# naver-ai/egtr

Hardware: AMD Instinct MI355X
Metric: images/sec end-to-end SGG, 600x1000 input, N=200 queries (higher is better)
Workload: dtype f32; 1 GPU; VG inference: ResNet-50, N=200, 6 enc/6 dec, 150 classes, 50 predicates, 600x1000, bs=1/GPU fp32 (BASELINE configs[1]); hip_graph=True, gemm_tuning=True, miopen_find=True, parallelism=replicas x1 (independent images, no collective)

## Files before the change

egtr_amd/csrc/ffn_x6.hip:

```cpp
#include <hip/hip_runtime.h>
#include <stdint.h>

#include "common.h"
#include "x6_common.h"
#include "xs_format.h"

namespace {
using namespace x6;

constexpr int kD = 256;
constexpr int kRows = 64;
constexpr int kKS = kD / 16;
constexpr int kFrag = xs::kFragBytes;
constexpr int kPanel = 2 * kKS * 2 * kFrag;
constexpr int kHbuf = 2 * 4 * 3 * kFrag;
constexpr int kStage = 24 * kFrag;
constexpr int kLds = kPanel + kHbuf + 3 * kStage;
static_assert(kLds == 160 * 1024, "the whole LDS of a CU");
constexpr int NL = 6;
typedef float f32x8 __attribute__((ext_vector_type(8)));

struct FfnArgs {
  const float* x;
  const float* res;
  const char* w1;
  const float* b1;
  const char* w2;
  const float* b2;
  const float* gamma;
  const float* beta;
  const float* pos;
  float* out;
  float* out_pos;
  int M, ldx, ldr, F, pos_rows;
  float eps;
  const char* wp;
  const float* bp;
  const float* gamma1;
  const float* beta1;
  float eps1;
};

__device__ __forceinline__ int swz(int x, int ks) { return x ^ (ks & 15) ^ ((x >> 5) << 2); }

__device__ __forceinline__ void build_panel(const float* __restrict__ x, int ldx, int M, int r0, int tid, int lane,
                                            char* panel, char* lo0, char* lo1) {
  float4 v[16];
#pragma unroll
  for (int it = 0; it < 16; ++it) {
    const int row = min(r0 + it * 4 + (tid >> 6), M - 1);
    v[it] = *reinterpret_cast<const float4*>(x + (size_t)row * ldx + 4 * lane);
  }
#pragma unroll
  for (int it = 0; it < 16; ++it) {
    const int row = it * 4 + (tid >> 6), rb = row >> 5, r = row & 31;
    const int ks = lane >> 2, off = (swz(r + 32 * ((lane >> 1) & 1), ks) << 4) + (lane & 1) * 8;
    const xs::Split3 s0 = xs::split3_fast(v[it].x), s1 = xs::split3_fast(v[it].y), s2 = xs::split3_fast(v[it].z),
                     s3 = xs::split3_fast(v[it].w);
    char* p = panel + ((rb * kKS + ks) * 2) * kFrag + off;
    *reinterpret_cast<uint2*>(p) = make_uint2(xs::pack_hi16(s0.hi, s1.hi), xs::pack_hi16(s2.hi, s3.hi));
    *reinterpret_cast<uint2*>(p + kFrag) = make_uint2(xs::pack_hi16(s0.mid, s1.mid), xs::pack_hi16(s2.mid, s3.mid));
    char* q = (rb == 0 ? lo0 : lo1) + ks * kFrag + off;
    *reinterpret_cast<uint2*>(q) = make_uint2(xs::pack_hi16(s0.lo, s1.lo), xs::pack_hi16(s2.lo, s3.lo));
  }
}

template <bool USE_RES_OF, class ResFn>
__device__ __forceinline__ void final_epilogue(const f32x16 (&acc2)[4], const FfnArgs& A, int r0, int wave, int lane,
                                               float* red, ResFn&& res_of) {
  const int wm = wave >> 1, wn = wave & 1, li = lane & 31, hf = lane >> 5;
  const int row = r0 + wm * 32 + li;
  float4 y[4][4];
#pragma unroll
  for (int t = 0; t < 4; ++t)
#pragma unroll
    for (int q = 0; q < 4; ++q) {
      const int col = (4 * wn + t) * 32 + 8 * q + 4 * hf;
      const float4 b = A.b2 != nullptr ? *reinterpret_cast<const float4*>(A.b2 + col) : make_float4(0.f, 0.f, 0.f, 0.f);
      y[t][q] = make_float4(acc2[t][4 * q + 0] + b.x, acc2[t][4 * q + 1] + b.y, acc2[t][4 * q + 2] + b.z,
                            acc2[t][4 * q + 3] + b.w);
    }
  if (A.gamma != nullptr) {
    const float* xr = A.res + (size_t)min(row, A.M - 1) * A.ldr;
#pragma unroll
    for (int t = 0; t < 4; ++t)
#pragma unroll
      for (int q = 0; q < 4; ++q) {
        float4 r;
        if constexpr (USE_RES_OF) r = res_of(t, q);
        else r = *reinterpret_cast<const float4*>(xr + (4 * wn + t) * 32 + 8 * q + 4 * hf);
        y[t][q].x += r.x; y[t][q].y += r.y; y[t][q].z += r.z; y[t][q].w += r.w;
      }
    __syncthreads();
    float sum = 0.f;
#pragma unroll
    for (int t = 0; t < 4; ++t)
#pragma unroll
      for (int q = 0; q < 4; ++q) sum += (y[t][q].x + y[t][q].y) + (y[t][q].z + y[t][q].w);
    sum += __shfl_xor(sum, 32);
    if (hf == 0) red[wave * 32 + li] = sum;
    __syncthreads();
    const float mean = (sum + red[(wave ^ 1) * 32 + li]) * (1.f / kD);
    float sq = 0.f;
#pragma unroll
    for (int t = 0; t < 4; ++t)
#pragma unroll
      for (int q = 0; q < 4; ++q) {
        y[t][q].x -= mean; y[t][q].y -= mean; y[t][q].z -= mean; y[t][q].w -= mean;
        sq += (y[t][q].x * y[t][q].x + y[t][q].y * y[t][q].y) + (y[t][q].z * y[t][q].z + y[t][q].w * y[t][q].w);
      }
    sq += __shfl_xor(sq, 32);
    if (hf == 0) red[128 + wave * 32 + li] = sq;
    __syncthreads();
    const float rstd = rsqrtf((sq + red[128 + (wave ^ 1) * 32 + li]) * (1.f / kD) + A.eps);
    const float* pr = A.out_pos != nullptr ? A.pos + (size_t)(min(row, A.M - 1) % A.pos_rows) * kD : nullptr;
#pragma unroll
    for (int t = 0; t < 4; ++t)
#pragma unroll
      for (int q = 0; q < 4; ++q) {
        const int col = (4 * wn + t) * 32 + 8 * q + 4 * hf;
        const float4 g = *reinterpret_cast<const float4*>(A.gamma + col), b = *reinterpret_cast<const float4*>(A.beta + col);
        y[t][q] = make_float4(y[t][q].x * rstd * g.x + b.x, y[t][q].y * rstd * g.y + b.y, y[t][q].z * rstd * g.z + b.z,
                              y[t][q].w * rstd * g.w + b.w);
        if (pr != nullptr && row < A.M) {
          const float4 p = *reinterpret_cast<const float4*>(pr + col);
          *reinterpret_cast<float4*>(A.out_pos + (size_t)row * kD + col) =
              make_float4(y[t][q].x + p.x, y[t][q].y + p.y, y[t][q].z + p.z, y[t][q].w + p.w);
        }
      }
  }
  if (row < A.M) {
#pragma unroll
    for (int t = 0; t < 4; ++t)
#pragma unroll
      for (int q = 0; q < 4; ++q)
        *reinterpret_cast<float4*>(A.out + (size_t)row * kD + (4 * wn + t) * 32 + 8 * q + 4 * hf) = y[t][q];
  }
}

__device__ __forceinline__ void layernorm_rows(float4 (&y)[4][4], const float* gamma, const float* beta, float eps, int wave,
                                               int lane, float* red) {
  const int wn = wave & 1, li = lane & 31, hf = lane >> 5;
  __syncthreads();
  float sum = 0.f;
#pragma unroll
  for (int t = 0; t < 4; ++t)
#pragma unroll
    for (int q = 0; q < 4; ++q) sum += (y[t][q].x + y[t][q].y) + (y[t][q].z + y[t][q].w);
  sum += __shfl_xor(sum, 32);
  if (hf == 0) red[wave * 32 + li] = sum;
  __syncthreads();
  const float mean = (sum + red[(wave ^ 1) * 32 + li]) * (1.f / kD);
  float sq = 0.f;
#pragma unroll
  for (int t = 0; t < 4; ++t)
#pragma unroll
    for (int q = 0; q < 4; ++q) {
      y[t][q].x -= mean; y[t][q].y -= mean; y[t][q].z -= mean; y[t][q].w -= mean;
      sq += (y[t][q].x * y[t][q].x + y[t][q].y * y[t][q].y) + (y[t][q].z * y[t][q].z + y[t][q].w * y[t][q].w);
    }
  sq += __shfl_xor(sq, 32);
  if (hf == 0) red[128 + wave * 32 + li] = sq;
  __syncthreads();
  const float rstd = rsqrtf((sq + red[128 + (wave ^ 1) * 32 + li]) * (1.f / kD) + eps);
#pragma unroll
  for (int t = 0; t < 4; ++t)
#pragma unroll
    for (int q = 0; q < 4; ++q) {
      const int col = (4 * wn + t) * 32 + 8 * q + 4 * hf;
      const float4 g = *reinterpret_cast<const float4*>(gamma + col), b = *reinterpret_cast<const float4*>(beta + col);
      y[t][q] = make_float4(y[t][q].x * rstd * g.x + b.x, y[t][q].y * rstd * g.y + b.y, y[t][q].z * rstd * g.z + b.z,
                            y[t][q].w * rstd * g.w + b.w);
    }
}

template <bool PROJ>
__global__ __launch_bounds__(256, 1) void ffn_x6_kernel(FfnArgs A) {
  extern __shared__ __attribute__((aligned(16))) char smem[];
  char* const panel = smem;
  char* const hbuf = smem + kPanel;
  char* const ring = smem + kPanel + kHbuf;
  const int tid = threadIdx.x, lane = tid & 63;
  const int wave = __builtin_amdgcn_readfirstlane(tid >> 6);
  const int wm = wave >> 1, wn = wave & 1;
  const int li = lane & 31, hf = lane >> 5;
  const unsigned lds_ring = (unsigned)reinterpret_cast<uintptr_t>((lds_char*)ring);
  const int r0 = blockIdx.x * kRows;
  const int nchunk = A.F >> 6, KSf = A.F >> 4;

  const unsigned voff = lane * 16;
  const int crot = blockIdx.x % nchunk;
  auto chunk_of = [&](int c) { const int t = c + crot; return t >= nchunk ? t - nchunk : t; };
  constexpr int NP = PROJ ? kKS : 0;
  const int nstages = NP + 8 * nchunk;
  const size_t nb_stride = (size_t)KSf * 3 * kFrag;
  auto stage_src = [&](int g, const char*& base, size_t& stride) {
    g = g < nstages ? g : nstages - 1;
    const bool pj = g < NP;
    const int gg = g - NP, c = chunk_of(pj ? 0 : gg >> 3), st = gg & 7;
    const bool l1 = st < 4;
    const char* b1 = A.w1 + ((size_t)((2 * c + (wave >> 1)) * kKS + 4 * (st & 3) + 2 * (wave & 1)) * 3) * kFrag;
    const char* b2 = A.w2 + ((size_t)(2 * wave * KSf + 4 * c + (st & 3)) * 3) * kFrag;
    base = l1 ? b1 : b2;
    stride = l1 ? (size_t)3 * kFrag : nb_stride;
    if constexpr (PROJ) {
      base = pj ? A.wp + ((size_t)(2 * wave * kKS + g) * 3) * kFrag : base;
      stride = pj ? (size_t)kKS * 3 * kFrag : stride;
    }
  };
  auto issue = [&](int g, int slot) {
    const unsigned dst = lds_ring + (unsigned)slot * kStage + (unsigned)wave * (NL * kFrag);
    const char* base;
    size_t stride;
    stage_src(g, base, stride);
#pragma unroll
    for (int i = 0; i < NL; ++i) dma16s(base + (i / 3) * stride + (i % 3) * kFrag, voff, dst + i * kFrag);
  };
  issue(0, 0);
  issue(1, 1);

  build_panel(A.x, A.ldx, A.M, r0, tid, lane, panel, hbuf, ring + 2 * kStage);
  __syncthreads();
  bf16x8 lo[kKS];
  {
    const char* q = (wm == 0 ? hbuf : ring + 2 * kStage);
#pragma unroll
    for (int ks = 0; ks < kKS; ++ks) lo[ks] = *reinterpret_cast<const bf16x8*>(q + ks * kFrag + (swz(lane, ks) << 4));
  }

  f32x16 acc2[4], acc1[2];
#pragma unroll
  for (int t = 0; t < 4; ++t)
#pragma unroll
    for (int r = 0; r < 16; ++r) acc2[t][r] = 0.f;

  auto pfrag = [&](int ks, int piece) {
    return *reinterpret_cast<const bf16x8*>(panel + ((wm * kKS + ks) * 2 + piece) * kFrag + (swz(lane, ks) << 4));
  };
  const char* const ph = hbuf + (wm * 4 * 3) * kFrag + lane * 16;
  const char* const pw = ring + (4 * wn * 3) * kFrag + lane * 16;
  auto frag = [](const char* p) { return *reinterpret_cast<const bf16x8*>(p); };

  auto stage = [&](auto S, const bf16x8 (&w)[4][3], bf16x8 (&wnx)[4][3], const bf16x8 (&a)[4][2], bf16x8 (&anx)[4][2], int g,
                   int slot_next, int slot_fill) {
    constexpr int s = decltype(S)::value;
    const char* const wn_src = pw + slot_next * kStage;
    const unsigned dst = lds_ring + (unsigned)slot_fill * kStage + (unsigned)wave * (NL * kFrag);
    const char* src;
    size_t sstride;
    stage_src(g + 3, src, sstride);
    static_for<24>([&](auto I) {
      constexpr int i = decltype(I)::value;
      constexpr int pwt[6] = {2, 0, 1, 1, 0, 0}, pat[6] = {0, 2, 1, 0, 1, 0};
      if constexpr (s < 4) {
        constexpr int pair = i / 12, term = (i % 12) / 2, par = i & 1, kl = 2 * pair + par;
        if constexpr (pat[term] == 2) acc1[par] = mfma(w[kl][pwt[term]], lo[4 * s + kl], acc1[par]);
        else acc1[par] = mfma(w[kl][pwt[term]], a[kl][pat[term]], acc1[par]);
        __builtin_amdgcn_sched_barrier(0);
      } else {
        constexpr int term = i / 4, t = i % 4;
        constexpr int ap = pat[term];
        acc2[t] = mfma(w[t][pwt[term]], a[ap >> 1][ap & 1], acc2[t]);
        __builtin_amdgcn_sched_barrier(0);
      }
      if constexpr ((i & 1) && (i >> 1) < NL) {
        constexpr int j = i >> 1;
        dma16s(src + (j / 3) * sstride + (j % 3) * kFrag, voff, dst + j * kFrag);
        __builtin_amdgcn_sched_barrier(0);
      }
      if constexpr (i >= 12 && i < 18) {
        constexpr int j = 2 * (i - 12);
        wnx[j / 3][j % 3] = frag(wn_src + j * kFrag);
        wnx[(j + 1) / 3][(j + 1) % 3] = frag(wn_src + (j + 1) * kFrag);
        __builtin_amdgcn_sched_barrier(0);
      }
      if constexpr (s < 8) {
        constexpr int sx = (s + 1) & 7;
        if constexpr (i >= 18 && i < 22 && sx < 4) {
          constexpr int kl = i - 18;
          anx[kl][0] = pfrag(4 * sx + kl, 0);
          anx[kl][1] = pfrag(4 * sx + kl, 1);
          __builtin_amdgcn_sched_barrier(0);
        }
        if constexpr (i == 18 && sx > 4) {
          anx[0][0] = frag(ph + ((sx - 4) * 3 + 0) * kFrag);
          anx[0][1] = frag(ph + ((sx - 4) * 3 + 1) * kFrag);
          anx[1][0] = frag(ph + ((sx - 4) * 3 + 2) * kFrag);
          __builtin_amdgcn_sched_barrier(0);
        }
      } else if constexpr (s - 8 + 1 < kKS) {
        if constexpr (i == 18) {
          anx[0][0] = pfrag(s - 8 + 1, 0);
          anx[0][1] = pfrag(s - 8 + 1, 1);
          anx[1][0] = lo[s - 8 + 1];
          __builtin_amdgcn_sched_barrier(0);
        }
      }
    });
  };

  bf16x8 w0[4][3], w1[4][3], a0[4][2], a1[4][2];
  f32x8 bias[4];
  wait_vm<NL>();
  wait_lgkm0();
  __builtin_amdgcn_s_barrier();
  issue(2, 2);
#pragma unroll
  for (int u = 0; u < 4; ++u)
#pragma unroll
    for (int p = 0; p < 3; ++p) w0[u][p] = frag(pw + (u * 3 + p) * kFrag);
  int slot = 0;
  int g = 0;
  auto stage_top = [&]() {
    wait_vm<NL>();
    wait_lgkm0();
    __builtin_amdgcn_s_barrier();
    __builtin_amdgcn_sched_barrier(0);
  };

  float4 y1[4][4];
  if constexpr (PROJ) {
    a0[0][0] = pfrag(0, 0);
    a0[0][1] = pfrag(0, 1);
    a0[1][0] = lo[0];
    static_for<kKS>([&](auto KS) {
      constexpr int ks = decltype(KS)::value;
      const int sn = slot == 2 ? 0 : slot + 1;
      stage_top();
      if constexpr ((ks & 1) == 0) stage(std::integral_constant<int, 8 + ks>{}, w0, w1, a0, a1, g, sn, slot);
      else stage(std::integral_constant<int, 8 + ks>{}, w1, w0, a1, a0, g, sn, slot);
      slot = sn;
      ++g;
    });
    const int row = r0 + wm * 32 + li;
    const float* xr = A.res + (size_t)min(row, A.M - 1) * A.ldr;
#pragma unroll
    for (int t = 0; t < 4; ++t)
#pragma unroll
      for (int q = 0; q < 4; ++q) {
        const int col = (4 * wn + t) * 32 + 8 * q + 4 * hf;
        const float4 b = *reinterpret_cast<const float4*>(A.bp + col), r = *reinterpret_cast<const float4*>(xr + col);
        y1[t][q] = make_float4(acc2[t][4 * q + 0] + b.x + r.x, acc2[t][4 * q + 1] + b.y + r.y, acc2[t][4 * q + 2] + b.z + r.z,
                               acc2[t][4 * q + 3] + b.w + r.w);
        acc2[t][4 * q + 0] = 0.f; acc2[t][4 * q + 1] = 0.f; acc2[t][4 * q + 2] = 0.f; acc2[t][4 * q + 3] = 0.f;
      }
    float* red = reinterpret_cast<float*>(hbuf + 16 * kFrag);
    layernorm_rows(y1, A.gamma1, A.beta1, A.eps1, wave, lane, red);
    uint2 plo[4][4];
#pragma unroll
    for (int t = 0; t < 4; ++t)
#pragma unroll
      for (int q = 0; q < 4; ++q) {
        const xs::Split3 s0 = xs::split3_fast(y1[t][q].x), s1 = xs::split3_fast(y1[t][q].y), s2 = xs::split3_fast(y1[t][q].z),
                         s3 = xs::split3_fast(y1[t][q].w);
        const int ks = 2 * (4 * wn + t) + (q >> 1);
        char* d = panel + ((wm * kKS + ks) * 2) * kFrag + (swz(li + 32 * (q & 1), ks) << 4) + 8 * hf;
        *reinterpret_cast<uint2*>(d) = make_uint2(xs::pack_hi16(s0.hi, s1.hi), xs::pack_hi16(s2.hi, s3.hi));
        *reinterpret_cast<uint2*>(d + kFrag) = make_uint2(xs::pack_hi16(s0.mid, s1.mid), xs::pack_hi16(s2.mid, s3.mid));
        plo[t][q] = make_uint2(xs::pack_hi16(s0.lo, s1.lo), xs::pack_hi16(s2.lo, s3.lo));
      }
#pragma unroll
    for (int rb = 0; rb < 2; ++rb) {
      if (wm == rb) {
#pragma unroll
        for (int t = 0; t < 4; ++t)
#pragma unroll
          for (int q = 0; q < 4; ++q) {
            const int ks = 2 * (4 * wn + t) + (q >> 1);
            *reinterpret_cast<uint2*>(hbuf + ks * kFrag + (swz(li + 32 * (q & 1), ks) << 4) + 8 * hf) = plo[t][q];
          }
      }
      __syncthreads();
      if (wm == rb) {
#pragma unroll
        for (int ks = 0; ks < kKS; ++ks) lo[ks] = *reinterpret_cast<const bf16x8*>(hbuf + ks * kFrag + (swz(lane, ks) << 4));
      }
      __syncthreads();
    }
  }
#pragma unroll
  for (int u = 0; u < 4; ++u) {
    a0[u][0] = pfrag(u, 0);
    a0[u][1] = pfrag(u, 1);
  }
#pragma unroll 1
  for (int c = 0; c < nchunk; ++c) {
    static_for<8>([&](auto S) {
      constexpr int s = decltype(S)::value;
      const int sn = slot == 2 ? 0 : slot + 1;
      stage_top();
      if constexpr (s == 4) {
        a0[0][0] = frag(ph + 0 * kFrag);
        a0[0][1] = frag(ph + 1 * kFrag);
        a0[1][0] = frag(ph + 2 * kFrag);
        __builtin_amdgcn_sched_barrier(0);
      }
      if constexpr (s == 0) {
#pragma unroll
        for (int t = 0; t < 2; ++t)
#pragma unroll
          for (int r = 0; r < 16; ++r) acc1[t][r] = 0.f;
        const float* bp = A.b1 + 64 * chunk_of(c) + 32 * wn;
        asm volatile("s_load_dwordx8 %0, %4, 0x0\n\ts_load_dwordx8 %1, %4, 0x20\n\ts_load_dwordx8 %2, %4, 0x40\n\t"
                     "s_load_dwordx8 %3, %4, 0x60"
                     : "=&s"(bias[0]), "=&s"(bias[1]), "=&s"(bias[2]), "=&s"(bias[3])
                     : "s"(bp));
      }
      if constexpr ((s & 1) == 0) stage(S, w0, w1, a0, a1, g, sn, slot);
      else stage(S, w1, w0, a1, a0, g, sn, slot);
      if constexpr (s == 3) {
        asm volatile("s_waitcnt lgkmcnt(0)" : "+s"(bias[0]), "+s"(bias[1]), "+s"(bias[2]), "+s"(bias[3]));
#pragma unroll
        for (int q = 0; q < 4; ++q) {
          float h[4];
#pragma unroll
          for (int j = 0; j < 4; ++j) {
            const float blo = bias[q][j], bhi = bias[q][4 + j];
            h[j] = egtr_relu(acc1[0][4 * q + j] + acc1[1][4 * q + j] + (hf ? bhi : blo));
          }
          char* dst = hbuf + ((wm * 4 + 2 * wn + (q >> 1)) * 3) * kFrag + (q & 1) * 512 + li * 16 + hf * 8;
          const xs::Split3 s0 = xs::split3_fast(h[0]), s1 = xs::split3_fast(h[1]), s2 = xs::split3_fast(h[2]),
                           s3 = xs::split3_fast(h[3]);
          *reinterpret_cast<uint2*>(dst) = make_uint2(xs::pack_hi16(s0.hi, s1.hi), xs::pack_hi16(s2.hi, s3.hi));
          *reinterpret_cast<uint2*>(dst + kFrag) = make_uint2(xs::pack_hi16(s0.mid, s1.mid), xs::pack_hi16(s2.mid, s3.mid));
          *reinterpret_cast<uint2*>(dst + 2 * kFrag) = make_uint2(xs::pack_hi16(s0.lo, s1.lo), xs::pack_hi16(s2.lo, s3.lo));
        }
      }
      slot = sn;
      ++g;
    });
  }
  wait_vm<0>();
  final_epilogue<PROJ>(acc2, A, r0, wave, lane, reinterpret_cast<float*>(ring), [&](int t, int q) { return y1[t][q]; });
  asm volatile("s_waitcnt vmcnt(0)" ::: "memory");
}


__global__ __launch_bounds__(256, 1) void proj_x6_kernel(FfnArgs A) {
  extern __shared__ __attribute__((aligned(16))) char smem[];
  char* const panel = smem;
  char* const ring = smem + kPanel;
  const int tid = threadIdx.x, lane = tid & 63;
  const int wave = __builtin_amdgcn_readfirstlane(tid >> 6);
  const int wm = wave >> 1, wn = wave & 1;
  const unsigned lds_ring = (unsigned)reinterpret_cast<uintptr_t>((lds_char*)ring);
  const int r0 = blockIdx.x * kRows;
  const unsigned voff = lane * 16;
  const int nw = A.F;
  auto src_of = [&](int w, int ks, int j) {
    if (ks >= kKS) { ks -= kKS; ++w; }
    if (w >= nw) { w = nw - 1; ks = kKS - 1; }
    return A.w2 + ((size_t)((8 * w + 2 * wave + j / 3) * kKS + ks) * 3 + j % 3) * kFrag;
  };
  auto issue = [&](int ks, int slot) {
    const unsigned dst = lds_ring + (unsigned)slot * kStage + (unsigned)wave * (NL * kFrag);
#pragma unroll
    for (int i = 0; i < NL; ++i) dma16s(src_of(0, ks, i), voff, dst + i * kFrag);
  };
  issue(0, 0);
  issue(1, 1);
  build_panel(A.x, A.ldx, A.M, r0, tid, lane, panel, ring + 2 * kStage, ring + 2 * kStage + kKS * kFrag);
  __syncthreads();
  bf16x8 lo[kKS];
  {
    const char* q = ring + 2 * kStage + wm * (kKS * kFrag);
#pragma unroll
    for (int ks = 0; ks < kKS; ++ks) lo[ks] = *reinterpret_cast<const bf16x8*>(q + ks * kFrag + (swz(lane, ks) << 4));
  }
  auto pfrag = [&](int ks, int piece) {
    return *reinterpret_cast<const bf16x8*>(panel + ((wm * kKS + ks) * 2 + piece) * kFrag + (swz(lane, ks) << 4));
  };
  const char* const pw = ring + (4 * wn * 3) * kFrag + lane * 16;
  auto frag = [](const char* p) { return *reinterpret_cast<const bf16x8*>(p); };
  bf16x8 w0[4][3], w1[4][3];
  wait_vm<NL>();
  wait_lgkm0();
  __builtin_amdgcn_s_barrier();
  issue(2, 2);
#pragma unroll
  for (int u = 0; u < 4; ++u)
#pragma unroll
    for (int p = 0; p < 3; ++p) w0[u][p] = frag(pw + (u * 3 + p) * kFrag);
  bf16x8 ahi = pfrag(0, 0), amid = pfrag(0, 1);
  int slot = 0;
#pragma unroll 1
  for (int w = 0; w < nw; ++w) {
    f32x16 acc2[4];
#pragma unroll
    for (int t = 0; t < 4; ++t)
#pragma unroll
      for (int r = 0; r < 16; ++r) acc2[t][r] = 0.f;
    static_for<kKS>([&](auto S) {
      constexpr int ks = decltype(S)::value;
      const int sn = slot == 2 ? 0 : slot + 1;
      wait_vm<NL>();
      wait_lgkm0();
      __builtin_amdgcn_s_barrier();
      __builtin_amdgcn_sched_barrier(0);
      const bf16x8 (&wc)[4][3] = (ks & 1) ? w1 : w0;
      bf16x8 (&wnx)[4][3] = (ks & 1) ? w0 : w1;
      const bf16x8 a0 = ahi, a1 = amid;
      const unsigned dst = lds_ring + (unsigned)slot * kStage + (unsigned)wave * (NL * kFrag);
      const char* const wn_src = pw + sn * kStage;
      static_for<24>([&](auto I) {
        constexpr int i = decltype(I)::value;
        constexpr int pwt[6] = {2, 0, 1, 1, 0, 0}, pat[6] = {0, 2, 1, 0, 1, 0};
        constexpr int term = i / 4, t = i % 4;
        if constexpr (pat[term] == 2) acc2[t] = mfma(wc[t][pwt[term]], lo[ks], acc2[t]);
        else acc2[t] = mfma(wc[t][pwt[term]], pat[term] == 0 ? a0 : a1, acc2[t]);
        __builtin_amdgcn_sched_barrier(0);
        if constexpr ((i & 1) && (i >> 1) < NL) {
          dma16s(src_of(w, ks + 3, i >> 1), voff, dst + (i >> 1) * kFrag);
          __builtin_amdgcn_sched_barrier(0);
        }
        if constexpr (i >= 12 && i < 18) {
          constexpr int j = 2 * (i - 12);
          wnx[j / 3][j % 3] = frag(wn_src + j * kFrag);
          wnx[(j + 1) / 3][(j + 1) % 3] = frag(wn_src + (j + 1) * kFrag);
          __builtin_amdgcn_sched_barrier(0);
        }
        if constexpr (i == 18) {
          ahi = pfrag((ks + 1) & (kKS - 1), 0);
          amid = pfrag((ks + 1) & (kKS - 1), 1);
          __builtin_amdgcn_sched_barrier(0);
        }
      });
      slot = sn;
    });
    FfnArgs Aw = A;
    Aw.out = A.out + (size_t)w * A.M * kD;
    Aw.b2 = A.b2 != nullptr ? A.b2 + w * kD : nullptr;
    if (w + 1 == nw) wait_vm<0>();
    final_epilogue<false>(acc2, Aw, r0, wave, lane, reinterpret_cast<float*>(ring), [](int, int) { return float4{}; });
  }
}

}

extern "C" int egtr_ffn_x6_f32(egtr_stream_t stream, const float* x, int ldx, const void* w1_xs, const float* b1,
                               const void* w2_xs, const float* b2, const float* ln_gamma, const float* ln_beta, float eps,
                               const float* pos, int pos_rows, float* out, float* out_pos, int M, int d_model, int ffn_dim) {
  if (!x || !w1_xs || !b1 || !w2_xs || !b2 || !out || M <= 0 || ldx < d_model) return EGTR_E_ARG;
  if ((ln_gamma == nullptr) != (ln_beta == nullptr) || (out_pos && (!pos || pos_rows <= 0 || !ln_gamma))) return EGTR_E_ARG;
  if (d_model != kD || ffn_dim <= 0 || ffn_dim % 64 || (ldx & 3) || (reinterpret_cast<uintptr_t>(x) & 15) ||
      (reinterpret_cast<uintptr_t>(out) & 15) || (reinterpret_cast<uintptr_t>(w1_xs) & 15) ||
      (reinterpret_cast<uintptr_t>(w2_xs) & 15) || (reinterpret_cast<uintptr_t>(b2) & 15) ||
      (out_pos && (reinterpret_cast<uintptr_t>(out_pos) & 15)) || (pos && (reinterpret_cast<uintptr_t>(pos) & 15)))
    return EGTR_E_UNSUPPORTED;
  static unsigned long long lds_raised = 0;
  if (int st = egtr_raise_dynamic_lds(reinterpret_cast<const void*>(ffn_x6_kernel<false>), kLds, &lds_raised)) return st;
  FfnArgs a{x, x, static_cast<const char*>(w1_xs), b1, static_cast<const char*>(w2_xs), b2, ln_gamma, ln_beta, pos, out,
            out_pos, M, ldx, ldx, ffn_dim, pos_rows, eps, nullptr, nullptr, nullptr, nullptr, 0.f};
  hipLaunchKernelGGL(ffn_x6_kernel<false>, dim3((M + kRows - 1) / kRows), dim3(256), kLds, static_cast<hipStream_t>(stream), a);
  return egtr_check_launch();
}

extern "C" int egtr_encoder_tail_x6_f32(egtr_stream_t stream, const float* context, int ldc, const float* hidden, int ldh,
                                        const void* wp_xs, const float* bp, const float* ln1_gamma, const float* ln1_beta,
                                        float eps1, const void* w1_xs, const float* b1, const void* w2_xs, const float* b2,
                                        const float* ln2_gamma, const float* ln2_beta, float eps2, const float* pos,
                                        int pos_rows, float* out, float* out_pos, int M, int d_model, int ffn_dim) {
  if (!context || !hidden || !wp_xs || !bp || !ln1_gamma || !ln1_beta || !w1_xs || !b1 || !w2_xs || !b2 || !ln2_gamma ||
      !ln2_beta || !out || M <= 0 || ldc < d_model || ldh < d_model)
    return EGTR_E_ARG;
  if (out_pos && (!pos || pos_rows <= 0)) return EGTR_E_ARG;
  if (d_model != kD || ffn_dim <= 0 || ffn_dim % 64 || (ldc & 3) || (ldh & 3)) return EGTR_E_UNSUPPORTED;
  for (const void* p : {(const void*)context, (const void*)hidden, wp_xs, (const void*)bp, (const void*)ln1_gamma,
                        (const void*)ln1_beta, w1_xs, w2_xs, (const void*)b2, (const void*)ln2_gamma, (const void*)ln2_beta,
                        (const void*)out, (const void*)out_pos, (const void*)pos})
    if (reinterpret_cast<uintptr_t>(p) & 15) return EGTR_E_UNSUPPORTED;
  static unsigned long long lds_raised = 0;
  if (int st = egtr_raise_dynamic_lds(reinterpret_cast<const void*>(ffn_x6_kernel<true>), kLds, &lds_raised)) return st;
  FfnArgs a{context, hidden, static_cast<const char*>(w1_xs), b1, static_cast<const char*>(w2_xs), b2, ln2_gamma, ln2_beta,
            pos, out, out_pos, M, ldc, ldh, ffn_dim, pos_rows, eps2, static_cast<const char*>(wp_xs), bp, ln1_gamma,
            ln1_beta, eps1};
  hipLaunchKernelGGL(ffn_x6_kernel<true>, dim3((M + kRows - 1) / kRows), dim3(256), kLds, static_cast<hipStream_t>(stream), a);
  return egtr_check_launch();
}

extern "C" int egtr_proj_ln_x6_f32(egtr_stream_t stream, const float* x, int ldx, const void* w_xs, const float* bias,
                                   const float* residual, int ldr, const float* ln_gamma, const float* ln_beta, float eps,
                                   const float* pos, int pos_rows, float* out, float* out_pos, int M, int d_model) {
  if (!x || !w_xs || !bias || !out || M <= 0 || ldx < d_model) return EGTR_E_ARG;
  if ((ln_gamma == nullptr) != (ln_beta == nullptr) || (ln_gamma && (!residual || ldr < d_model)) ||
      (out_pos && (!pos || pos_rows <= 0 || !ln_gamma)))
    return EGTR_E_ARG;
  if (d_model != kD || (ldx & 3) || (ldr & 3) || (reinterpret_cast<uintptr_t>(x) & 15) ||
      (reinterpret_cast<uintptr_t>(out) & 15) || (reinterpret_cast<uintptr_t>(w_xs) & 15) ||
      (reinterpret_cast<uintptr_t>(bias) & 15) || (reinterpret_cast<uintptr_t>(residual) & 15) ||
      (out_pos && (reinterpret_cast<uintptr_t>(out_pos) & 15)) || (pos && (reinterpret_cast<uintptr_t>(pos) & 15)))
    return EGTR_E_UNSUPPORTED;
  constexpr int lds = kPanel + 3 * kStage + 8 * kFrag;
  static unsigned long long lds_raised = 0;
  if (int st = egtr_raise_dynamic_lds(reinterpret_cast<const void*>(proj_x6_kernel), lds, &lds_raised)) return st;
  FfnArgs a{x, residual, nullptr, nullptr, static_cast<const char*>(w_xs), bias, ln_gamma, ln_beta, pos, out, out_pos,
            M, ldx, ldr, 1, pos_rows, eps};
  hipLaunchKernelGGL(proj_x6_kernel, dim3((M + kRows - 1) / kRows), dim3(256), lds, static_cast<hipStream_t>(stream), a);
  return egtr_check_launch();
}

extern "C" int egtr_proj_multi_x6_f32(egtr_stream_t stream, const float* x, int ldx, const void* w_xs, const float* bias,
                                      float* out, int M, int d_model, int num_weights) {
  if (!x || !w_xs || !out || M <= 0 || ldx < d_model || num_weights <= 0) return EGTR_E_ARG;
  if (d_model != kD || (ldx & 3) || (reinterpret_cast<uintptr_t>(x) & 15) || (reinterpret_cast<uintptr_t>(out) & 15) ||
      (reinterpret_cast<uintptr_t>(w_xs) & 15) || (bias && (reinterpret_cast<uintptr_t>(bias) & 15)))
    return EGTR_E_UNSUPPORTED;
  constexpr int lds = kPanel + 3 * kStage + 8 * kFrag;
  static unsigned long long lds_raised = 0;
  if (int st = egtr_raise_dynamic_lds(reinterpret_cast<const void*>(proj_x6_kernel), lds, &lds_raised)) return st;
  FfnArgs a{x, nullptr, nullptr, nullptr, static_cast<const char*>(w_xs), bias, nullptr, nullptr, nullptr, out, nullptr,
            M, ldx, 0, num_weights, 0, 0.f};
  hipLaunchKernelGGL(proj_x6_kernel, dim3((M + kRows - 1) / kRows), dim3(256), lds, static_cast<hipStream_t>(stream), a);
  return egtr_check_launch();
}
```

Measured before the change: 403.2 images/sec.

## Persistent split-unit scheduling for multi-weight projection kernel across CUs

```diff
diff --git a/egtr_amd/csrc/ffn_x6.hip b/egtr_amd/csrc/ffn_x6.hip
--- a/egtr_amd/csrc/ffn_x6.hip
+++ b/egtr_amd/csrc/ffn_x6.hip
@@ -1,6 +1,7 @@
 #include <hip/hip_runtime.h>
 #include <stdint.h>
 
+#include "../../include/egtr_hip_test_sched.h"
 #include "common.h"
 #include "x6_common.h"
 #include "xs_format.h"
@@ -43,14 +44,16 @@
 
 __device__ __forceinline__ int swz(int x, int ks) { return x ^ (ks & 15) ^ ((x >> 5) << 2); }
 
-__device__ __forceinline__ void build_panel(const float* __restrict__ x, int ldx, int M, int r0, int tid, int lane,
-                                            char* panel, char* lo0, char* lo1) {
-  float4 v[16];
+__device__ __forceinline__ void load_panel(const float* __restrict__ x, int ldx, int M, int r0, int tid, int lane,
+                                           float4 (&v)[16]) {
 #pragma unroll
   for (int it = 0; it < 16; ++it) {
     const int row = min(r0 + it * 4 + (tid >> 6), M - 1);
     v[it] = *reinterpret_cast<const float4*>(x + (size_t)row * ldx + 4 * lane);
   }
+}
+
+__device__ __forceinline__ void split_panel(const float4 (&v)[16], int tid, int lane, char* panel, char* lo0, char* lo1) {
 #pragma unroll
   for (int it = 0; it < 16; ++it) {
     const int row = it * 4 + (tid >> 6), rb = row >> 5, r = row & 31;
@@ -63,6 +66,13 @@
     char* q = (rb == 0 ? lo0 : lo1) + ks * kFrag + off;
     *reinterpret_cast<uint2*>(q) = make_uint2(xs::pack_hi16(s0.lo, s1.lo), xs::pack_hi16(s2.lo, s3.lo));
   }
+}
+
+__device__ __forceinline__ void build_panel(const float* __restrict__ x, int ldx, int M, int r0, int tid, int lane,
+                                            char* panel, char* lo0, char* lo1) {
+  float4 v[16];
+  load_panel(x, ldx, M, r0, tid, lane, v);
+  split_panel(v, tid, lane, panel, lo0, lo1);
 }
 
 template <bool USE_RES_OF, class ResFn>
@@ -444,94 +454,118 @@
   const int wave = __builtin_amdgcn_readfirstlane(tid >> 6);
   const int wm = wave >> 1, wn = wave & 1;
   const unsigned lds_ring = (unsigned)reinterpret_cast<uintptr_t>((lds_char*)ring);
-  const int r0 = blockIdx.x * kRows;
   const unsigned voff = lane * 16;
   const int nw = A.F;
+  const long long U = (long long)((A.M + kRows - 1) / kRows) * nw;
+  int u = (int)(blockIdx.x * U / gridDim.x);
+  const int u_end = (int)((blockIdx.x + 1) * U / gridDim.x);
+  int r0 = (u / nw) * kRows, w_lo = u % nw, w_hi = min(nw, w_lo + (u_end - u));
   auto src_of = [&](int w, int ks, int j) {
     if (ks >= kKS) { ks -= kKS; ++w; }
-    if (w >= nw) { w = nw - 1; ks = kKS - 1; }
+    if (w >= w_hi) { w = w_hi - 1; ks = kKS - 1; }
     return A.w2 + ((size_t)((8 * w + 2 * wave + j / 3) * kKS + ks) * 3 + j % 3) * kFrag;
   };
   auto issue = [&](int ks, int slot) {
     const unsigned dst = lds_ring + (unsigned)slot * kStage + (unsigned)wave * (NL * kFrag);
 #pragma unroll
-    for (int i = 0; i < NL; ++i) dma16s(src_of(0, ks, i), voff, dst + i * kFrag);
-  };
+    for (int i = 0; i < NL; ++i) dma16s(src_of(w_lo, ks, i), voff, dst + i * kFrag);
+  };
+  auto pfrag = [&](int ks, int piece) {
+    return *reinterpret_cast<const bf16x8*>(panel + ((wm * kKS + ks) * 2 + piece) * kFrag + (swz(lane, ks) << 4));
+  };
+  const char* const pw = ring + (4 * wn * 3) * kFrag + lane * 16;
+  auto frag = [](const char* p) { return *reinterpret_cast<const bf16x8*>(p); };
   issue(0, 0);
   issue(1, 1);
-  build_panel(A.x, A.ldx, A.M, r0, tid, lane, panel, ring + 2 * kStage, ring + 2 * kStage + kKS * kFrag);
-  __syncthreads();
-  bf16x8 lo[kKS];
-  {
-    const char* q = ring + 2 * kStage + wm * (kKS * kFrag);
-#pragma unroll
-    for (int ks = 0; ks < kKS; ++ks) lo[ks] = *reinterpret_cast<const bf16x8*>(q + ks * kFrag + (swz(lane, ks) << 4));
-  }
-  auto pfrag = [&](int ks, int piece) {
-    return *reinterpret_cast<const bf16x8*>(panel + ((wm * kKS + ks) * 2 + piece) * kFrag + (swz(lane, ks) << 4));
-  };
-  const char* const pw = ring + (4 * wn * 3) * kFrag + lane * 16;
-  auto frag = [](const char* p) { return *reinterpret_cast<const bf16x8*>(p); };
-  bf16x8 w0[4][3], w1[4][3];
-  wait_vm<NL>();
-  wait_lgkm0();
-  __builtin_amdgcn_s_barrier();
-  issue(2, 2);
-#pragma unroll
-  for (int u = 0; u < 4; ++u)
-#pragma unroll
-    for (int p = 0; p < 3; ++p) w0[u][p] = frag(pw + (u * 3 + p) * kFrag);
-  bf16x8 ahi = pfrag(0, 0), amid = pfrag(0, 1);
-  int slot = 0;
+  float4 xrows[16];
+  load_panel(A.x, A.ldx, A.M, r0, tid, lane, xrows);
 #pragma unroll 1
-  for (int w = 0; w < nw; ++w) {
-    f32x16 acc2[4];
-#pragma unroll
-    for (int t = 0; t < 4; ++t)
-#pragma unroll
-      for (int r = 0; r < 16; ++r) acc2[t][r] = 0.f;
-    static_for<kKS>([&](auto S) {
-      constexpr int ks = decltype(S)::value;
-      const int sn = slot == 2 ? 0 : slot + 1;
-      wait_vm<NL>();
-      wait_lgkm0();
-      __builtin_amdgcn_s_barrier();
-      __builtin_amdgcn_sched_barrier(0);
-      const bf16x8 (&wc)[4][3] = (ks & 1) ? w1 : w0;
-      bf16x8 (&wnx)[4][3] = (ks & 1) ? w0 : w1;
-      const bf16x8 a0 = ahi, a1 = amid;
-      const unsigned dst = lds_ring + (unsigned)slot * kStage + (unsigned)wave * (NL * kFrag);
-      const char* const wn_src = pw + sn * kStage;
-      static_for<24>([&](auto I) {
-        constexpr int i = decltype(I)::value;
-        constexpr int pwt[6] = {2, 0, 1, 1, 0, 0}, pat[6] = {0, 2, 1, 0, 1, 0};
-        constexpr int term = i / 4, t = i % 4;
-        if constexpr (pat[term] == 2) acc2[t] = mfma(wc[t][pwt[term]], lo[ks], acc2[t]);
-        else acc2[t] = mfma(wc[t][pwt[term]], pat[term] == 0 ? a0 : a1, acc2[t]);
+  for (;;) {
+    split_panel(xrows, tid, lane, panel, ring + 2 * kStage, ring + 2 * kStage + kKS * kFrag);
+    __syncthreads();
+    bf16x8 lo[kKS];
+    {
+      const char* q = ring + 2 * kStage + wm * (kKS * kFrag);
+#pragma unroll
+      for (int ks = 0; ks < kKS; ++ks) lo[ks] = *reinterpret_cast<const bf16x8*>(q + ks * kFrag + (swz(lane, ks) << 4));
+    }
+    bf16x8 w0[4][3], w1[4][3];
+    wait_vm<NL>();
+    wait_lgkm0();
+    __builtin_amdgcn_s_barrier();
+    issue(2, 2);
+#pragma unroll
+    for (int t = 0; t < 4; ++t)
+#pragma unroll
+      for (int p = 0; p < 3; ++p) w0[t][p] = frag(pw + (t * 3 + p) * kFrag);
+    bf16x8 ahi = pfrag(0, 0), amid = pfrag(0, 1);
+    int slot = 0;
+    u += w_hi - w_lo;
+    const bool more = u < u_end;
+#pragma unroll 1
+    for (int w = w_lo; w < w_hi; ++w) {
+      f32x16 acc2[4];
+#pragma unroll
+      for (int t = 0; t < 4; ++t)
+#pragma unroll
+        for (int r = 0; r < 16; ++r) acc2[t][r] = 0.f;
+      static_for<kKS>([&](auto S) {
+        constexpr int ks = decltype(S)::value;
+        const int sn = slot == 2 ? 0 : slot + 1;
+        wait_vm<NL>();
+        wait_lgkm0();
+        __builtin_amdgcn_s_barrier();
         __builtin_amdgcn_sched_barrier(0);
-        if constexpr ((i & 1) && (i >> 1) < NL) {
-          dma16s(src_of(w, ks + 3, i >> 1), voff, dst + (i >> 1) * kFrag);
+        const bf16x8 (&wc)[4][3] = (ks & 1) ? w1 : w0;
+        bf16x8 (&wnx)[4][3] = (ks & 1) ? w0 : w1;
+        const bf16x8 a0 = ahi, a1 = amid;
+        const unsigned dst = lds_ring + (unsigned)slot * kStage + (unsigned)wave * (NL * kFrag);
+        const char* const wn_src = pw + sn * kStage;
+        static_for<24>([&](auto I) {
+          constexpr int i = decltype(I)::value;
+          constexpr int pwt[6] = {2, 0, 1, 1, 0, 0}, pat[6] = {0, 2, 1, 0, 1, 0};
+          constexpr int term = i / 4, t = i % 4;
+          if constexpr (pat[term] == 2) acc2[t] = mfma(wc[t][pwt[term]], lo[ks], acc2[t]);
+          else acc2[t] = mfma(wc[t][pwt[term]], pat[term] == 0 ? a0 : a1, acc2[t]);
           __builtin_amdgcn_sched_barrier(0);
+          if constexpr ((i & 1) && (i >> 1) < NL) {
+            dma16s(src_of(w, ks + 3, i >> 1), voff, dst + (i >> 1) * kFrag);
+            __builtin_amdgcn_sched_barrier(0);
+          }
+          if constexpr (i >= 12 && i < 18) {
+            constexpr int j = 2 * (i - 12);
+            wnx[j / 3][j % 3] = frag(wn_src + j * kFrag);
+            wnx[(j + 1) / 3][(j + 1) % 3] = frag(wn_src + (j + 1) * kFrag);
+            __builtin_amdgcn_sched_barrier(0);
+          }
+          if constexpr (i == 18) {
+            ahi = pfrag((ks + 1) & (kKS - 1), 0);
+            amid = pfrag((ks + 1) & (kKS - 1), 1);
+            __builtin_amdgcn_sched_barrier(0);
+          }
+        });
+        slot = sn;
+      });
+      FfnArgs Aw = A;
+      Aw.out = A.out + (size_t)w * A.M * kD;
+      Aw.b2 = A.b2 != nullptr ? A.b2 + w * kD : nullptr;
+      const int rows_at = r0;
+      if (w + 1 == w_hi) {
+        wait_vm<0>();
+        if (more) {
+          r0 += kRows;
+          load_panel(A.x, A.ldx, A.M, r0, tid, lane, xrows);
         }
-        if constexpr (i >= 12 && i < 18) {
-          constexpr int j = 2 * (i - 12);
-          wnx[j / 3][j % 3] = frag(wn_src + j * kFrag);
-          wnx[(j + 1) / 3][(j + 1) % 3] = frag(wn_src + (j + 1) * kFrag);
-          __builtin_amdgcn_sched_barrier(0);
-        }
-        if constexpr (i == 18) {
-          ahi = pfrag((ks + 1) & (kKS - 1), 0);
-          amid = pfrag((ks + 1) & (kKS - 1), 1);
-          __builtin_amdgcn_sched_barrier(0);
-        }
-      });
-      slot = sn;
-    });
-    FfnArgs Aw = A;
-    Aw.out = A.out + (size_t)w * A.M * kD;
-    Aw.b2 = A.b2 != nullptr ? A.b2 + w * kD : nullptr;
-    if (w + 1 == nw) wait_vm<0>();
-    final_epilogue<false>(acc2, Aw, r0, wave, lane, reinterpret_cast<float*>(ring), [](int, int) { return float4{}; });
+      }
+      final_epilogue<false>(acc2, Aw, rows_at, wave, lane, reinterpret_cast<float*>(ring), [](int, int) { return float4{}; });
+    }
+    if (!more) break;
+    w_lo = 0;
+    w_hi = min(nw, u_end - u);
+    wait_lgkm0();
+    __builtin_amdgcn_s_barrier();
+    issue(0, 0);
+    issue(1, 1);
   }
 }
 
@@ -599,17 +633,51 @@
   return egtr_check_launch();
 }
 
-extern "C" int egtr_proj_multi_x6_f32(egtr_stream_t stream, const float* x, int ldx, const void* w_xs, const float* bias,
-                                      float* out, int M, int d_model, int num_weights) {
+namespace {
+int cu_count() {
+  static int cus[64] = {};
+  int dev = 0;
+  if (hipGetDevice(&dev) != hipSuccess || dev < 0) return 0;
+  int& n = cus[dev & 63];
+  int got = __atomic_load_n(&n, __ATOMIC_ACQUIRE);
+  if (got == 0) {
+    if (hipDeviceGetAttribute(&got, hipDeviceAttributeMultiprocessorCount, dev) != hipSuccess || got <= 0) return 0;
+    __atomic_store_n(&n, got, __ATOMIC_RELEASE);
+  }
+  return got;
+}
+
+int launch_proj_multi(egtr_stream_t stream, const float* x, int ldx, const void* w_xs, const float* bias, float* out, int M,
+                      int d_model, int num_weights, int workgroups) {
   if (!x || !w_xs || !out || M <= 0 || ldx < d_model || num_weights <= 0) return EGTR_E_ARG;
+  const long long units = (long long)((M + kRows - 1) / kRows) * num_weights;
+  if (workgroups < 0 || workgroups > units) return EGTR_E_ARG;
   if (d_model != kD || (ldx & 3) || (reinterpret_cast<uintptr_t>(x) & 15) || (reinterpret_cast<uintptr_t>(out) & 15) ||
-      (reinterpret_cast<uintptr_t>(w_xs) & 15) || (bias && (reinterpret_cast<uintptr_t>(bias) & 15)))
+      (reinterpret_cast<uintptr_t>(w_xs) & 15) || (bias && (reinterpret_cast<uintptr_t>(bias) & 15)) || units > INT32_MAX)
     return EGTR_E_UNSUPPORTED;
+  if (workgroups == 0) {
+    const int cus = cu_count();
+    if (cus <= 0) return egtr_check_launch();
+    workgroups = (int)(units < cus ? units : cus);
+  }
   constexpr int lds = kPanel + 3 * kStage + 8 * kFrag;
   static unsigned long long lds_raised = 0;
   if (int st = egtr_raise_dynamic_lds(reinterpret_cast<const void*>(proj_x6_kernel), lds, &lds_raised)) return st;
   FfnArgs a{x, nullptr, nullptr, nullptr, static_cast<const char*>(w_xs), bias, nullptr, nullptr, nullptr, out, nullptr,
             M, ldx, 0, num_weights, 0, 0.f};
-  hipLaunchKernelGGL(proj_x6_kernel, dim3((M + kRows - 1) / kRows), dim3(256), lds, static_cast<hipStream_t>(stream), a);
+  hipLaunchKernelGGL(proj_x6_kernel, dim3(workgroups), dim3(256), lds, static_cast<hipStream_t>(stream), a);
   return egtr_check_launch();
 }
+}
+
+extern "C" int egtr_proj_multi_x6_f32(egtr_stream_t stream, const float* x, int ldx, const void* w_xs, const float* bias,
+                                      float* out, int M, int d_model, int num_weights) {
+  return launch_proj_multi(stream, x, ldx, w_xs, bias, out, M, d_model, num_weights, 0);
+}
+
+extern "C" int egtr_test_proj_multi_x6_f32_grid(egtr_stream_t stream, const float* x, int ldx, const void* w_xs,
+                                                const float* bias, float* out, int M, int d_model, int num_weights,
+                                                int workgroups) {
+  if (workgroups < 1) return EGTR_E_ARG;
+  return launch_proj_multi(stream, x, ldx, w_xs, bias, out, M, d_model, num_weights, workgroups);
+}
diff --git a/include/egtr_hip_test_sched.h b/include/egtr_hip_test_sched.h
--- /dev/null
+++ b/include/egtr_hip_test_sched.h
@@ -0,0 +1,16 @@
+#ifndef EGTR_HIP_TEST_SCHED_H
+#define EGTR_HIP_TEST_SCHED_H
+
+#include "egtr_hip.h"
+
+#ifdef __cplusplus
+extern "C" {
+#endif
+
+int egtr_test_proj_multi_x6_f32_grid(egtr_stream_t stream, const float* x, int ldx, const void* w_xs, const float* bias,
+                                     float* out, int M, int d_model, int num_weights, int workgroups);
+
+#ifdef __cplusplus
+}
+#endif
+#endif
```

New measurement: 405.2 images/sec, median of 6. Within noise of the previous version (+0.5%).
